# camlab-ethz/poseidon

Hardware: AMD Instinct MI355X
Metric: PDE-grid samples/sec (fwd+bwd) (higher is better)
Workload: dtype fp16

## Files before the change

poseidon_amd/csrc/wgrad_mlp.hip:

```cpp
#include "wgrad_group.h"
#include <stdlib.h>

typedef unsigned int u32x4_t __attribute__((ext_vector_type(4)));

struct WgradMlpArgs {
  const bf16_t* h16; const bf16_t* dz;
  const bf16_t* W1; const float* b1;
  const bf16_t* W2T;
  float* ws;
  size_t plane;
  int M, hid, rows_per_slice, nslice, use_tr;
  int nslice_launch;
};

template <int C, int HT> struct WgradMlpLds {
  static constexpr int HW = 64 * HT, PW = C + 8, TK = 32;
  static constexpr size_t bytes = (size_t)(2 * HW * PW + 2 * TK * PW) * 2;
};

template <int C, int HT>
__global__ __launch_bounds__(256, 2) void wgrad_mlp_kernel(WgradMlpArgs p) {
  constexpr int KJ = C / 32, CT = C / 16, HW = 64 * HT, PW = C + 8, TK = 32;
  constexpr int NW = HW * C / 8, PWN = NW / 256;
  constexpr int NT = TK * C / 8, PTN = (NT + 255) / 256;
  static_assert(NW % 256 == 0, "weight chunk pieces must divide over the 256 threads");
  __shared__ __attribute__((aligned(16))) char smem[WgradMlpLds<C, HT>::bytes];
  bf16_t* W1c = (bf16_t*)smem;
  bf16_t* W2c = W1c + HW * PW;
  bf16_t* Ht = W2c + HW * PW;
  bf16_t* Dt = Ht + TK * PW;
  const int tid = threadIdx.x, lane = tid & 63, wave = tid >> 6, g = lane >> 4, lc = lane & 15;
  const int hid = p.hid, nchunk = hid / HW;
  int L = blockIdx.x, slice, chunk;
  if (p.nslice_launch % 8 == 0) { const int j = L >> 3; slice = (L & 7) * (p.nslice_launch >> 3) + j / nchunk; chunk = j % nchunk; }
  else { slice = L / nchunk; chunk = L % nchunk; }
  if (slice >= p.nslice) return;
  const int row_beg = slice * p.rows_per_slice, row_end = min(p.M, row_beg + p.rows_per_slice);

  {
    const bf16_t* s1 = p.W1 + (size_t)chunk * HW * C;
    const bf16_t* s2 = p.W2T + (size_t)chunk * HW * C;
    u32x4_t r1[PWN], r2[PWN];
#pragma unroll
    for (int u = 0; u < PWN; ++u) { r1[u] = *(const u32x4_t*)(s1 + (size_t)(tid + u * 256) * 8); r2[u] = *(const u32x4_t*)(s2 + (size_t)(tid + u * 256) * 8); }
#pragma unroll
    for (int u = 0; u < PWN; ++u) {
      const int i = tid + u * 256;
      *(u32x4_t*)(W1c + (i / (C / 8)) * PW + (i % (C / 8)) * 8) = r1[u];
      *(u32x4_t*)(W2c + (i / (C / 8)) * PW + (i % (C / 8)) * 8) = r2[u];
    }
  }
  float bias[HT];
#pragma unroll
  for (int hh = 0; hh < HT; ++hh) bias[hh] = p.b1[chunk * HW + (wave * HT + hh) * 16 + lc];

  f32x4_t aW1[HT][CT], aW2[HT][CT];
  float sdu[HT];
#pragma unroll
  for (int hh = 0; hh < HT; ++hh) {
    sdu[hh] = 0.f;
#pragma unroll
    for (int ct = 0; ct < CT; ++ct) { aW1[hh][ct] = (f32x4_t){0.f, 0.f, 0.f, 0.f}; aW2[hh][ct] = (f32x4_t){0.f, 0.f, 0.f, 0.f}; }
  }
  float sdz = 0.f;

  u32x4_t rh[PTN], rd[PTN];
  auto load_rows = [&](int r0) {
#pragma unroll
    for (int u = 0; u < PTN; ++u) {
      const int i = min(tid + u * 256, NT - 1);
      const int row = min(r0 + i / (C / 8), p.M - 1);
      const size_t o = (size_t)row * C + (i % (C / 8)) * 8;
      rh[u] = *(const u32x4_t*)(p.h16 + o);
      rd[u] = *(const u32x4_t*)(p.dz + o);
    }
  };
  auto store_rows = [&](int r0) {
#pragma unroll
    for (int u = 0; u < PTN; ++u) {
      const int i = tid + u * 256;
      if (i < NT) {
        const int tr = i / (C / 8);
        const bool ok = r0 + tr < row_end;
        const u32x4_t z = {0u, 0u, 0u, 0u};
        *(u32x4_t*)(Ht + tr * PW + (i % (C / 8)) * 8) = ok ? rh[u] : z;
        *(u32x4_t*)(Dt + tr * PW + (i % (C / 8)) * 8) = ok ? rd[u] : z;
      }
    }
  };
  const int nsteps = (p.rows_per_slice + TK - 1) / TK;
  load_rows(row_beg);
  for (int st = 0; st < nsteps; ++st) {
    const int r0 = row_beg + st * TK;
    __syncthreads();
    store_rows(r0);
    __syncthreads();
    load_rows(r0 + TK);
    if (chunk == 0 && tid < C) {
#pragma unroll 8
      for (int t = 0; t < TK; ++t) sdz += bf2f(Dt[t * PW + tid]);
    }
    f32x4_t U[HT][2], D[HT][2];
#pragma unroll
    for (int hh = 0; hh < HT; ++hh)
#pragma unroll
      for (int tt = 0; tt < 2; ++tt) { U[hh][tt] = (f32x4_t){0.f, 0.f, 0.f, 0.f}; D[hh][tt] = (f32x4_t){0.f, 0.f, 0.f, 0.f}; }
#pragma unroll
    for (int j = 0; j < KJ; ++j) {
      Frag<bf16_t> w1[HT], w2[HT];
#pragma unroll
      for (int hh = 0; hh < HT; ++hh) {
        w1[hh] = lds_frag_kc(W1c, PW, (wave * HT + hh) * 16, j * 32, lane);
        w2[hh] = lds_frag_kc(W2c, PW, (wave * HT + hh) * 16, j * 32, lane);
      }
#pragma unroll
      for (int tt = 0; tt < 2; ++tt) {
        const Frag<bf16_t> hA = lds_frag_kc(Ht, PW, tt * 16, j * 32, lane), dA = lds_frag_kc(Dt, PW, tt * 16, j * 32, lane);
#pragma unroll
        for (int hh = 0; hh < HT; ++hh) { mma16(U[hh][tt], hA, w1[hh]); mma16(D[hh][tt], dA, w2[hh]); }
      }
    }
    Frag<bf16_t> actf[HT], duf[HT];
#pragma unroll
    for (int hh = 0; hh < HT; ++hh) {
      float av[8], dv[8];
#pragma unroll
      for (int tt = 0; tt < 2; ++tt)
#pragma unroll
        for (int r = 0; r < 4; ++r) {
          const float x = U[hh][tt][r] + bias[hh];
          float cdf, e;
          gelu_terms(x, cdf, e);
          av[4 * tt + r] = x * cdf;
          dv[4 * tt + r] = D[hh][tt][r] * bf2f(f2bf(cdf + x * 0.3989422804014327f * e));
        }
      actf[hh] = frag_from_f32<bf16_t>(av);
      duf[hh] = frag_from_f32<bf16_t>(dv);
#pragma unroll
      for (int j = 0; j < 8; ++j) sdu[hh] += bf2f((bf16_t)duf[hh].v[j]);
    }
#pragma unroll
    for (int ct = 0; ct < CT; ++ct) {
      const Frag<bf16_t> hB = lds_frag_ks(Ht, PW, ct * 16, g * 4, 16 + g * 4, lane, p.use_tr);
      const Frag<bf16_t> dA = lds_frag_ks(Dt, PW, ct * 16, g * 4, 16 + g * 4, lane, p.use_tr);
#pragma unroll
      for (int hh = 0; hh < HT; ++hh) {
        mma16(aW1[hh][ct], duf[hh], hB);
        mma16(aW2[hh][ct], dA, actf[hh]);
      }
    }
  }

  float* pl = p.ws + (size_t)slice * p.plane;
  const size_t oW1 = 0, ob1 = (size_t)hid * C, oW2 = ob1 + hid, ob2 = oW2 + (size_t)C * hid;
#pragma unroll
  for (int hh = 0; hh < HT; ++hh) {
    const int hg = chunk * HW + (wave * HT + hh) * 16;
#pragma unroll
    for (int ct = 0; ct < CT; ++ct)
#pragma unroll
      for (int r = 0; r < 4; ++r) {
        pl[oW1 + (size_t)(hg + g * 4 + r) * C + ct * 16 + lc] = aW1[hh][ct][r];
        pl[oW2 + (size_t)(ct * 16 + g * 4 + r) * hid + hg + lc] = aW2[hh][ct][r];
      }
    float s = sdu[hh];
    s += __shfl_xor(s, 16, 64);
    s += __shfl_xor(s, 32, 64);
    if (g == 0) pl[ob1 + hg + lc] = s;
  }
  if (chunk == 0 && tid < C) pl[ob2 + tid] = sdz;
}

template <int ZL>
__global__ __launch_bounds__(256) void plane_reduce_kernel(const float* __restrict__ ws, float* __restrict__ grad, size_t plane, int nz,
                                                           size_t wlen, size_t w2beg, int mode, const float* scale) {
  const size_t n8 = plane / 8;
  const int zl = threadIdx.x % ZL;
  for (size_t i = ((size_t)blockIdx.x * blockDim.x + threadIdx.x) / ZL; i < n8; i += (size_t)gridDim.x * blockDim.x / ZL) {
    float acc[8];
#pragma unroll
    for (int j = 0; j < 8; ++j) acc[j] = 0.f;
#pragma unroll 4
    for (int z = zl; z < nz; z += ZL) {
      float v[8];
      ld8(ws + (size_t)z * plane, SCOT_F32, i * 8, v);
#pragma unroll
      for (int j = 0; j < 8; ++j) acc[j] += v[j];
    }
#pragma unroll
    for (int o = 1; o < ZL; o <<= 1)
#pragma unroll
      for (int j = 0; j < 8; ++j) acc[j] += __shfl_xor(acc[j], o, 64);
    if (zl == 0) {
      const size_t e = i * 8;
      const bool weight = e < wlen || (e >= w2beg && e < w2beg + wlen);
      grad_commit8(grad, e, acc, weight ? mode : SCOT_GRAD_ADD, scale);
    }
  }
}

extern int g_scot_use_tr;

static void wgrad_mlp_plan(int M, int C, int hid, int* nslice, int* rps) {
  const int want = C == 96 ? 256 : 512;
  const int hw = C == 96 ? 128 : 64, nchunk = hid / hw;
  int ns = (want + nchunk - 1) / nchunk;
  if (ns < 1) ns = 1;
  if (ns >= 8) ns = ns / 8 * 8;
  int r = ((M + ns - 1) / ns + 31) / 32 * 32;
  if (r < 256) r = 256;
  if (r > ((M + 31) / 32) * 32) r = ((M + 31) / 32) * 32;
  *rps = r;
  *nslice = (M + r - 1) / r;
}
static int round8(int n) { return n >= 8 ? (n + 7) / 8 * 8 : n; }

extern "C" size_t scot_wgrad_mlp_workspace_bytes(int M, int C, int hid) {
  if (M <= 0 || (C != 96 && C != 192) || hid != 4 * C) return 0;
  int ns, rps;
  wgrad_mlp_plan(M, C, hid, &ns, &rps);
  return (size_t)ns * ((size_t)2 * hid * C + hid + C) * sizeof(float);
}

extern "C" int scot_wgrad_mlp(const void* h16, const void* dz, const void* W1, const float* b1, const void* W2T, float* dW1, float* db1,
                              float* dW2, float* db2, int M, int C, int hid, void* workspace, size_t ws_bytes, int mode,
                              const float* grad_scale, hipStream_t stream) {
  if (M <= 0 || mode < 0 || mode > SCOT_GRAD_ADD_SCALED) return SCOT_ERR_SHAPE;
  if ((C != 96 && C != 192) || hid != 4 * C) return SCOT_ERR_UNSUPPORTED;
  if (!h16 || !dz || !W1 || !b1 || !W2T || !dW1 || !db1 || !dW2 || !db2 || !workspace) return SCOT_ERR_SHAPE;
  if (db1 != dW1 + (size_t)hid * C || dW2 != db1 + hid || db2 != dW2 + (size_t)C * hid) return SCOT_ERR_UNSUPPORTED;
  if ((((uintptr_t)h16 | (uintptr_t)dz | (uintptr_t)W1 | (uintptr_t)W2T | (uintptr_t)workspace | (uintptr_t)dW1) & 31) != 0) return SCOT_ERR_SHAPE;
  WgradMlpArgs a;
  a.h16 = (const bf16_t*)h16; a.dz = (const bf16_t*)dz; a.W1 = (const bf16_t*)W1; a.b1 = b1; a.W2T = (const bf16_t*)W2T;
  a.ws = (float*)workspace; a.M = M; a.hid = hid; a.use_tr = g_scot_use_tr;
  a.plane = (size_t)2 * hid * C + hid + C;
  wgrad_mlp_plan(M, C, hid, &a.nslice, &a.rows_per_slice);
  if ((size_t)a.nslice * a.plane * sizeof(float) > ws_bytes) return SCOT_ERR_SHAPE;
  const int nchunk = hid / (C == 96 ? 128 : 64);
  a.nslice_launch = round8(a.nslice);
  const dim3 grid((unsigned)(nchunk * a.nslice_launch)), block(256);
  if (C == 96) hipLaunchKernelGGL((wgrad_mlp_kernel<96, 2>), grid, block, 0, stream, a);
  else hipLaunchKernelGGL((wgrad_mlp_kernel<192, 1>), grid, block, 0, stream, a);
  int rc = scot_check_launch();
  if (rc != SCOT_OK) return rc;
  const size_t n8 = a.plane / 8;
  const int zl = a.nslice >= 32 ? 8 : a.nslice >= 4 ? 4 : 1;
  size_t blocks = (n8 * zl + 255) / 256; if (blocks > 2048) blocks = 2048;
  const dim3 gr((unsigned)blocks), b(256);
  const size_t wlen = (size_t)hid * C, w2beg = wlen + hid;
  if (zl == 8) hipLaunchKernelGGL(plane_reduce_kernel<8>, gr, b, 0, stream, a.ws, dW1, a.plane, a.nslice, wlen, w2beg, mode, grad_scale);
  else if (zl == 4) hipLaunchKernelGGL(plane_reduce_kernel<4>, gr, b, 0, stream, a.ws, dW1, a.plane, a.nslice, wlen, w2beg, mode, grad_scale);
  else hipLaunchKernelGGL(plane_reduce_kernel<1>, gr, b, 0, stream, a.ws, dW1, a.plane, a.nslice, wlen, w2beg, mode, grad_scale);
  return scot_check_launch();
}
```

Baseline: 3541.

## Double-buffer MLP wgrad row tiles, split rows across two wave halves

For C=96 the MLP weight-gradient kernel now runs 512 threads. Two groups of four waves each take half of a 64-row tile and share one copy of the weight chunk in LDS. Their partial accumulators are summed through LDS at the end. Row tiles are double-buffered, which halves barriers per step. The db2 column sum becomes an MFMA against a ones fragment spread across waves, and the plane reduce gains a 16-lane variant for many slices. The intent is better latency hiding and less serial per-thread work, at the cost of higher register and LDS pressure and a lower occupancy bound.

```diff
diff --git a/poseidon_amd/csrc/wgrad_mlp.hip b/poseidon_amd/csrc/wgrad_mlp.hip
--- a/poseidon_amd/csrc/wgrad_mlp.hip
+++ b/poseidon_amd/csrc/wgrad_mlp.hip
@@ -13,23 +13,28 @@
   int nslice_launch;
 };
 
-template <int C, int HT> struct WgradMlpLds {
-  static constexpr int HW = 64 * HT, PW = C + 8, TK = 32;
-  static constexpr size_t bytes = (size_t)(2 * HW * PW + 2 * TK * PW) * 2;
+template <int C, int HT, int NH, int NBUF> struct WgradMlpLds {
+  static constexpr int HW = 64 * HT, PW = C + 8, TK = 32 * NH;
+  static constexpr size_t wbytes = (size_t)2 * HW * PW * 2, tbytes = (size_t)2 * TK * PW * 2;
+  static constexpr size_t bytes = wbytes + NBUF * tbytes;
+  static constexpr int NRED = 2 * HT * (C / 16) * 4 + HT + 4;
+  static_assert(NH == 1 || NBUF == 2, "the half-to-half sum reuses LDS that the last step's barrier has released");
+  static_assert(NH == 1 || (size_t)NRED * 256 * 4 <= bytes, "the half-to-half sum must fit in the kernel's LDS");
 };
 
-template <int C, int HT>
-__global__ __launch_bounds__(256, 2) void wgrad_mlp_kernel(WgradMlpArgs p) {
-  constexpr int KJ = C / 32, CT = C / 16, HW = 64 * HT, PW = C + 8, TK = 32;
-  constexpr int NW = HW * C / 8, PWN = NW / 256;
-  constexpr int NT = TK * C / 8, PTN = (NT + 255) / 256;
-  static_assert(NW % 256 == 0, "weight chunk pieces must divide over the 256 threads");
-  __shared__ __attribute__((aligned(16))) char smem[WgradMlpLds<C, HT>::bytes];
+template <int C, int HT, int NH, int NBUF>
+__global__ __launch_bounds__(256 * NH, 2 / NH) void wgrad_mlp_kernel(WgradMlpArgs p) {
+  using Lds = WgradMlpLds<C, HT, NH, NBUF>;
+  constexpr int KJ = C / 32, CT = C / 16, HW = 64 * HT, PW = C + 8, TK = Lds::TK, NTH = 256 * NH;
+  constexpr int NW = HW * C / 8, PWN = NW / NTH;
+  constexpr int NT = TK * C / 8, PTN = (NT + NTH - 1) / NTH;
+  static_assert(NW % NTH == 0, "weight chunk pieces must divide over the threads");
+  __shared__ __attribute__((aligned(16))) char smem[Lds::bytes];
   bf16_t* W1c = (bf16_t*)smem;
   bf16_t* W2c = W1c + HW * PW;
-  bf16_t* Ht = W2c + HW * PW;
-  bf16_t* Dt = Ht + TK * PW;
+  bf16_t* ring = W2c + HW * PW;
   const int tid = threadIdx.x, lane = tid & 63, wave = tid >> 6, g = lane >> 4, lc = lane & 15;
+  const int wq = wave & 3, half = wave >> 2;
   const int hid = p.hid, nchunk = hid / HW;
   int L = blockIdx.x, slice, chunk;
   if (p.nslice_launch % 8 == 0) { const int j = L >> 3; slice = (L & 7) * (p.nslice_launch >> 3) + j / nchunk; chunk = j % nchunk; }
@@ -42,17 +47,17 @@
     const bf16_t* s2 = p.W2T + (size_t)chunk * HW * C;
     u32x4_t r1[PWN], r2[PWN];
 #pragma unroll
-    for (int u = 0; u < PWN; ++u) { r1[u] = *(const u32x4_t*)(s1 + (size_t)(tid + u * 256) * 8); r2[u] = *(const u32x4_t*)(s2 + (size_t)(tid + u * 256) * 8); }
+    for (int u = 0; u < PWN; ++u) { r1[u] = *(const u32x4_t*)(s1 + (size_t)(tid + u * NTH) * 8); r2[u] = *(const u32x4_t*)(s2 + (size_t)(tid + u * NTH) * 8); }
 #pragma unroll
     for (int u = 0; u < PWN; ++u) {
-      const int i = tid + u * 256;
+      const int i = tid + u * NTH;
       *(u32x4_t*)(W1c + (i / (C / 8)) * PW + (i % (C / 8)) * 8) = r1[u];
       *(u32x4_t*)(W2c + (i / (C / 8)) * PW + (i % (C / 8)) * 8) = r2[u];
     }
   }
   float bias[HT];
 #pragma unroll
-  for (int hh = 0; hh < HT; ++hh) bias[hh] = p.b1[chunk * HW + (wave * HT + hh) * 16 + lc];
+  for (int hh = 0; hh < HT; ++hh) bias[hh] = p.b1[chunk * HW + (wq * HT + hh) * 16 + lc];
 
   f32x4_t aW1[HT][CT], aW2[HT][CT];
   float sdu[HT];
@@ -62,44 +67,60 @@
 #pragma unroll
     for (int ct = 0; ct < CT; ++ct) { aW1[hh][ct] = (f32x4_t){0.f, 0.f, 0.f, 0.f}; aW2[hh][ct] = (f32x4_t){0.f, 0.f, 0.f, 0.f}; }
   }
-  float sdz = 0.f;
+  const int sct = chunk + nchunk * wq;
+  const bool has_sdz = sct < CT;
+  f32x4_t sdz = (f32x4_t){0.f, 0.f, 0.f, 0.f};
+  Frag<bf16_t> ones;
+#pragma unroll
+  for (int j = 0; j < 8; ++j) frag_set(ones, j, 1.f);
 
   u32x4_t rh[PTN], rd[PTN];
   auto load_rows = [&](int r0) {
 #pragma unroll
     for (int u = 0; u < PTN; ++u) {
-      const int i = min(tid + u * 256, NT - 1);
+      const int i = min(tid + u * NTH, NT - 1);
       const int row = min(r0 + i / (C / 8), p.M - 1);
       const size_t o = (size_t)row * C + (i % (C / 8)) * 8;
       rh[u] = *(const u32x4_t*)(p.h16 + o);
       rd[u] = *(const u32x4_t*)(p.dz + o);
     }
   };
-  auto store_rows = [&](int r0) {
+  auto store_rows = [&](bf16_t* buf, int r0) {
 #pragma unroll
     for (int u = 0; u < PTN; ++u) {
-      const int i = tid + u * 256;
+      const int i = tid + u * NTH;
       if (i < NT) {
         const int tr = i / (C / 8);
         const bool ok = r0 + tr < row_end;
         const u32x4_t z = {0u, 0u, 0u, 0u};
-        *(u32x4_t*)(Ht + tr * PW + (i % (C / 8)) * 8) = ok ? rh[u] : z;
-        *(u32x4_t*)(Dt + tr * PW + (i % (C / 8)) * 8) = ok ? rd[u] : z;
+        *(u32x4_t*)(buf + tr * PW + (i % (C / 8)) * 8) = ok ? rh[u] : z;
+        *(u32x4_t*)(buf + (TK + tr) * PW + (i % (C / 8)) * 8) = ok ? rd[u] : z;
       }
     }
   };
   const int nsteps = (p.rows_per_slice + TK - 1) / TK;
   load_rows(row_beg);
+  if constexpr (NBUF == 2) {
+    store_rows(ring, row_beg);
+    load_rows(row_beg + TK);
+    __syncthreads();
+  }
   for (int st = 0; st < nsteps; ++st) {
     const int r0 = row_beg + st * TK;
-    __syncthreads();
-    store_rows(r0);
-    __syncthreads();
-    load_rows(r0 + TK);
-    if (chunk == 0 && tid < C) {
-#pragma unroll 8
-      for (int t = 0; t < TK; ++t) sdz += bf2f(Dt[t * PW + tid]);
-    }
+    bf16_t* cur = ring + (NBUF == 2 ? (st & 1) * (2 * TK * PW) : 0);
+    if constexpr (NBUF == 2) {
+      if (st + 1 < nsteps) {
+        store_rows(ring + ((st + 1) & 1) * (2 * TK * PW), r0 + TK);
+        load_rows(r0 + 2 * TK);
+      }
+    } else {
+      __syncthreads();
+      store_rows(ring, r0);
+      __syncthreads();
+      load_rows(r0 + TK);
+    }
+    const bf16_t* Ht = cur + half * 32 * PW;
+    const bf16_t* Dt = cur + (TK + half * 32) * PW;
     f32x4_t U[HT][2], D[HT][2];
 #pragma unroll
     for (int hh = 0; hh < HT; ++hh)
@@ -110,8 +131,8 @@
       Frag<bf16_t> w1[HT], w2[HT];
 #pragma unroll
       for (int hh = 0; hh < HT; ++hh) {
-        w1[hh] = lds_frag_kc(W1c, PW, (wave * HT + hh) * 16, j * 32, lane);
-        w2[hh] = lds_frag_kc(W2c, PW, (wave * HT + hh) * 16, j * 32, lane);
+        w1[hh] = lds_frag_kc(W1c, PW, (wq * HT + hh) * 16, j * 32, lane);
+        w2[hh] = lds_frag_kc(W2c, PW, (wq * HT + hh) * 16, j * 32, lane);
       }
 #pragma unroll
       for (int tt = 0; tt < 2; ++tt) {
@@ -120,6 +141,7 @@
         for (int hh = 0; hh < HT; ++hh) { mma16(U[hh][tt], hA, w1[hh]); mma16(D[hh][tt], dA, w2[hh]); }
       }
     }
+    if (has_sdz) mma16(sdz, lds_frag_ks(Dt, PW, sct * 16, g * 4, 16 + g * 4, lane, p.use_tr), ones);
     Frag<bf16_t> actf[HT], duf[HT];
 #pragma unroll
     for (int hh = 0; hh < HT; ++hh) {
@@ -149,13 +171,46 @@
         mma16(aW2[hh][ct], dA, actf[hh]);
       }
     }
+    if constexpr (NBUF == 2) __syncthreads();
+  }
+  if constexpr (NH == 2) {
+    float* red = (float*)smem;
+    const int t4 = tid & 255;
+    if (half == 1) {
+      int v = 0;
+#pragma unroll
+      for (int hh = 0; hh < HT; ++hh) {
+#pragma unroll
+        for (int ct = 0; ct < CT; ++ct)
+#pragma unroll
+          for (int r = 0; r < 4; ++r) { red[(v++) * 256 + t4] = aW1[hh][ct][r]; red[(v++) * 256 + t4] = aW2[hh][ct][r]; }
+        red[(v++) * 256 + t4] = sdu[hh];
+      }
+#pragma unroll
+      for (int r = 0; r < 4; ++r) red[(v++) * 256 + t4] = sdz[r];
+    }
+    __syncthreads();
+    if (half == 1) return;
+    {
+      int v = 0;
+#pragma unroll
+      for (int hh = 0; hh < HT; ++hh) {
+#pragma unroll
+        for (int ct = 0; ct < CT; ++ct)
+#pragma unroll
+          for (int r = 0; r < 4; ++r) { aW1[hh][ct][r] += red[(v++) * 256 + t4]; aW2[hh][ct][r] += red[(v++) * 256 + t4]; }
+        sdu[hh] += red[(v++) * 256 + t4];
+      }
+#pragma unroll
+      for (int r = 0; r < 4; ++r) sdz[r] += red[(v++) * 256 + t4];
+    }
   }
 
   float* pl = p.ws + (size_t)slice * p.plane;
   const size_t oW1 = 0, ob1 = (size_t)hid * C, oW2 = ob1 + hid, ob2 = oW2 + (size_t)C * hid;
 #pragma unroll
   for (int hh = 0; hh < HT; ++hh) {
-    const int hg = chunk * HW + (wave * HT + hh) * 16;
+    const int hg = chunk * HW + (wq * HT + hh) * 16;
 #pragma unroll
     for (int ct = 0; ct < CT; ++ct)
 #pragma unroll
@@ -168,7 +223,10 @@
     s += __shfl_xor(s, 32, 64);
     if (g == 0) pl[ob1 + hg + lc] = s;
   }
-  if (chunk == 0 && tid < C) pl[ob2 + tid] = sdz;
+  if (has_sdz && lc == 0) {
+#pragma unroll
+    for (int r = 0; r < 4; ++r) pl[ob2 + sct * 16 + g * 4 + r] = sdz[r];
+  }
 }
 
 template <int ZL>
@@ -202,14 +260,14 @@
 extern int g_scot_use_tr;
 
 static void wgrad_mlp_plan(int M, int C, int hid, int* nslice, int* rps) {
-  const int want = C == 96 ? 256 : 512;
+  const int want = C == 96 ? 256 : 512, tk = C == 96 ? 64 : 32;
   const int hw = C == 96 ? 128 : 64, nchunk = hid / hw;
   int ns = (want + nchunk - 1) / nchunk;
   if (ns < 1) ns = 1;
   if (ns >= 8) ns = ns / 8 * 8;
-  int r = ((M + ns - 1) / ns + 31) / 32 * 32;
+  int r = ((M + ns - 1) / ns + tk - 1) / tk * tk;
   if (r < 256) r = 256;
-  if (r > ((M + 31) / 32) * 32) r = ((M + 31) / 32) * 32;
+  if (r > ((M + tk - 1) / tk) * tk) r = ((M + tk - 1) / tk) * tk;
   *rps = r;
   *nslice = (M + r - 1) / r;
 }
@@ -238,17 +296,18 @@
   if ((size_t)a.nslice * a.plane * sizeof(float) > ws_bytes) return SCOT_ERR_SHAPE;
   const int nchunk = hid / (C == 96 ? 128 : 64);
   a.nslice_launch = round8(a.nslice);
-  const dim3 grid((unsigned)(nchunk * a.nslice_launch)), block(256);
-  if (C == 96) hipLaunchKernelGGL((wgrad_mlp_kernel<96, 2>), grid, block, 0, stream, a);
-  else hipLaunchKernelGGL((wgrad_mlp_kernel<192, 1>), grid, block, 0, stream, a);
+  const dim3 grid((unsigned)(nchunk * a.nslice_launch));
+  if (C == 96) hipLaunchKernelGGL((wgrad_mlp_kernel<96, 2, 2, 2>), grid, dim3(512), 0, stream, a);
+  else hipLaunchKernelGGL((wgrad_mlp_kernel<192, 1, 1, 1>), grid, dim3(256), 0, stream, a);
   int rc = scot_check_launch();
   if (rc != SCOT_OK) return rc;
   const size_t n8 = a.plane / 8;
-  const int zl = a.nslice >= 32 ? 8 : a.nslice >= 4 ? 4 : 1;
+  const int zl = a.nslice >= 64 ? 16 : a.nslice >= 32 ? 8 : a.nslice >= 4 ? 4 : 1;
   size_t blocks = (n8 * zl + 255) / 256; if (blocks > 2048) blocks = 2048;
   const dim3 gr((unsigned)blocks), b(256);
   const size_t wlen = (size_t)hid * C, w2beg = wlen + hid;
-  if (zl == 8) hipLaunchKernelGGL(plane_reduce_kernel<8>, gr, b, 0, stream, a.ws, dW1, a.plane, a.nslice, wlen, w2beg, mode, grad_scale);
+  if (zl == 16) hipLaunchKernelGGL(plane_reduce_kernel<16>, gr, b, 0, stream, a.ws, dW1, a.plane, a.nslice, wlen, w2beg, mode, grad_scale);
+  else if (zl == 8) hipLaunchKernelGGL(plane_reduce_kernel<8>, gr, b, 0, stream, a.ws, dW1, a.plane, a.nslice, wlen, w2beg, mode, grad_scale);
   else if (zl == 4) hipLaunchKernelGGL(plane_reduce_kernel<4>, gr, b, 0, stream, a.ws, dW1, a.plane, a.nslice, wlen, w2beg, mode, grad_scale);
   else hipLaunchKernelGGL(plane_reduce_kernel<1>, gr, b, 0, stream, a.ws, dW1, a.plane, a.nslice, wlen, w2beg, mode, grad_scale);
   return scot_check_launch();
```

New measurement: 3542, median of 6. About the same (+0.0%).
